# cgtuebingen/3D-RE-GEN

Hardware: AMD Instinct MI355X
Metric: objects/sec (50-step Hunyuan3D-2 DiT + 256^3 marching cubes) (higher is better)
Workload: dtype bf16; 1 GPU; configs[1]: 5 synthetic 512x512 RGBA crops per GPU, Hunyuan3D-2 full dims bf16, 50 flow-matching steps x CFG 2, 257^3 grid query + Lewiner marching cubes; weights=seeded synthetic, objects_total=5, objects_per_launch=4, parallelism=object-parallel x1

## Files before the change

3d-re-gen_amd/csrc/attn.hip:

```cpp
#include <hip/hip_runtime.h>
#include <cstdio>
#include <cstring>
#include <stddef.h>
#include <stdint.h>

#include <type_traits>

#include "kernels.h"
#include "prof.h"

namespace r3g {
namespace {

typedef __attribute__((ext_vector_type(8))) __bf16 bf16x8;
typedef __attribute__((ext_vector_type(4))) __bf16 bf16x4;
typedef __attribute__((ext_vector_type(16))) float f32x16;
typedef __attribute__((ext_vector_type(8))) float f32x8;

constexpr int KV_TILE = 64;
constexpr int TILE_B = KV_TILE * 64 * 2;
constexpr int STAGE_B = 2 * TILE_B;

typedef __attribute__((ext_vector_type(2))) __bf16 bf16x2;
typedef __attribute__((ext_vector_type(2))) float f32x2;
// ... 791 lines not shown
                m_run = half_max(mx);
#pragma unroll
                for (int r = 0; r < 16; ++r) { negm[r] = -m_run; s[r] -= m_run; }
            } else if (!kFast && __any(q < Lq && !(mx <= SCORE_LIMIT))) {
                const float grow = fmaxf(half_max(mx), 0.f);
                const float alpha = __builtin_amdgcn_exp2f(-grow);
                m_run += grow;
                l_run *= alpha;
#pragma unroll
                for (int r = 0; r < 16; ++r) { o[0][r] *= alpha; o[1][r] *= alpha; negm[r] -= grow; s[r] -= grow; }
            }
            float pe[16];
            uint32_t pk[8];
#pragma unroll
            for (int r = 0; r < 16; ++r) pe[r] = (ABL & 1) ? s[r] * 0.001f : __builtin_amdgcn_exp2f(s[r]);
#pragma unroll
            for (int e = 0; e < 8; ++e) pk[e] = pack_bf16(pe[2 * e], pe[2 * e + 1]);
            {
                const float psum = sum16(pe);
                l_run += psum;
                if (kFast && !first_block) sticky |= __ballot(!(psum <= PSUM_LIMIT2)) & valid_lanes;
            }
#pragma unroll
            for (int ks2 = 0; ks2 < 2; ++ks2) {
                union { uint32_t u[4]; bf16x8 v; } pf;
#pragma unroll
                for (int e = 0; e < 4; ++e) pf.u[e] = pk[4 * ks2 + e];
#pragma unroll
                for (int db = 0; db < 2; ++db) {
                    const bf16x8 vf = (ABL & 64) ? qf[(ks2 + db) & 3]
                                                 : *reinterpret_cast<const bf16x8*>(cur + TILE_B + (off[db] ^ ((2 * kb + ks2) << 5)));
                    if (ABL & 4) asm volatile("" ::"v"(vf), "v"(pf.v));
                    else o[db] = __builtin_amdgcn_mfma_f32_32x32x16_bf16(vf, pf.v, o[db], 0, 0, 0);
                }
            }
        }
        if (!(ABL & 32)) {
            asm volatile("s_waitcnt vmcnt(0)" ::: "memory");
            __syncthreads();
        }
    };
    if (ntiles == 1) {
        if (pad_tail) tile(std::true_type{}, std::true_type{}, 0);
        else tile(std::false_type{}, std::true_type{}, 0);
    } else {
        tile(std::false_type{}, std::true_type{}, 0);
        for (int t = 1; t < ntiles - 1; ++t) tile(std::false_type{}, std::false_type{}, t);
        if (pad_tail) tile(std::true_type{}, std::false_type{}, ntiles - 1);
        else tile(std::false_type{}, std::false_type{}, ntiles - 1);
    }
    };
    if constexpr ((VAR & 1) != 0 && ABL == 0) {
        pass(std::true_type{});
        if (__syncthreads_or(sticky != 0)) pass(std::false_type{});
    } else {
        pass(std::false_type{});
    }
    }

    const float inv = 1.0f / half_sum(l_run);
    {
        int64_t orow = (int64_t)b * p.strideO + (int64_t)q * p.ldo;
        if (p.ragged) orow = attn_entry_out_row(eb, q) * p.ldo;
        uint16_t* dst = p.O + orow + hd * 64;
#pragma unroll
        for (int db = 0; db < 2; ++db)
#pragma unroll
            for (int gp = 0; gp < 2; ++gp) {
                uint2 even, odd;
                even.x = pack_bf16(o[db][8 * gp] * inv, o[db][8 * gp + 1] * inv);
                even.y = pack_bf16(o[db][8 * gp + 2] * inv, o[db][8 * gp + 3] * inv);
                odd.x = pack_bf16(o[db][8 * gp + 4] * inv, o[db][8 * gp + 5] * inv);
                odd.y = pack_bf16(o[db][8 * gp + 6] * inv, o[db][8 * gp + 7] * inv);
                const u32x2 rx = __builtin_amdgcn_permlane32_swap(even.x, odd.x, false, false);
                const u32x2 ry = __builtin_amdgcn_permlane32_swap(even.y, odd.y, false, false);
                uint4 out;
                out.x = rx[0]; out.y = ry[0]; out.z = rx[1]; out.w = ry[1];
                if (q < Lq) *reinterpret_cast<uint4*>(dst + db * 32 + 16 * gp + 8 * hh) = out;
            }
    }
}

struct SoftmaxRun { float ps0, ps1, ea, eb; };
template <int J>
__device__ __forceinline__ void softmax_step(f32x8& half, uint32_t (&pk)[8], SoftmaxRun& st) {
    asm volatile("" : "+v"(half));
    const float a = __builtin_amdgcn_exp2f(half[2 * (J & 3)]);
    const float b = __builtin_amdgcn_exp2f(half[2 * (J & 3) + 1]);
    if (J == 1) { st.ps0 = st.ea; st.ps1 = st.eb; }
    if (J > 1) { st.ps0 += st.ea; st.ps1 += st.eb; }
    if (J > 0) {
        pk[J - 1] = pack_bf16(st.ea, st.eb);
        asm volatile("" : "+v"(pk[J - 1]));
    }
    st.ea = a;
    st.eb = b;
    if (J == 7) {
        pk[7] = pack_bf16(a, b);
        st.ps0 += a;
        st.ps1 += b;
        asm volatile("" : "+v"(pk[7]));
    }
    asm volatile("" : "+v"(st.ps0), "+v"(st.ps1), "+v"(st.ea), "+v"(st.eb));
}

template <int NW, int VAR = 0>
__global__ __launch_bounds__(NW * 64, 2) void attn3_kernel(AttnArgs p) {
    __shared__ __attribute__((aligned(16))) char smem[2 * STAGE_B];
    const int tid = threadIdx.x, lane = tid & 63;
    const int wid = __builtin_amdgcn_readfirstlane(tid >> 6);
    const int ql = lane & 31, hh = lane >> 5;
    constexpr int QT = NW * 64;
    int eb, hd, qt;
    {
        const int nwg = gridDim.x, orig = blockIdx.x;
        const int qn = nwg >> 3, rn = nwg & 7, xcd = orig & 7;
        const int item = (xcd < rn ? xcd * (qn + 1) : rn * (qn + 1) + (xcd - rn) * qn) + (orig >> 3);
        attn_work_item<QT>(p, item, eb, hd, qt);
    }
    const AttnEntry en = attn_entry(p, eb);
    const int b = en.buf;
    const int q0 = qt * QT + wid * 64 + ql;
    const int Lq = en.lq, Lk = en.lk;
    const int kvb = p.kv_batch_stride_zero ? 0 : b;
    const uint16_t* Qg = p.Q + (((int64_t)b * p.H + hd) * p.Lq_pad) * 64;
    const uint16_t* Kg = p.K + (((int64_t)kvb * p.H + hd) * p.Lk_pad) * 64;
    const uint16_t* Vtg = p.Vt + (((int64_t)kvb * p.H + hd) * 64) * (int64_t)p.Lk_pad;

    bf16x8 qf[2][4];
#pragma unroll
    for (int qb = 0; qb < 2; ++qb) {
        const int q = q0 + qb * 32;
        const int qrow = q < p.Lq_pad ? q : p.Lq_pad - 1;
#pragma unroll
        for (int ks = 0; ks < 4; ++ks)
            qf[qb][ks] = *reinterpret_cast<const bf16x8*>(Qg + (int64_t)qrow * 64 + ks * 16 + hh * 8);
    }
    if (!p.q_prescaled) {
        const float sc = p.scale * 1.4426950408889634f;
#pragma unroll
        for (int qb = 0; qb < 2; ++qb)
#pragma unroll
            for (int ks = 0; ks < 4; ++ks) {
                union { bf16x8 v; uint32_t u[4]; } w;
                w.v = qf[qb][ks];
#pragma unroll
                for (int e = 0; e < 4; ++e)
                    w.u[e] = pack_bf16(__uint_as_float(w.u[e] << 16) * sc, __uint_as_float(w.u[e] & 0xFFFF0000u) * sc);
                qf[qb][ks] = w.v;
            }
    }

    f32x16 o[2][2], negm[2];
    float m_run[2], l_run[2];
    unsigned long long sticky = 0;
    const unsigned long long valid_lanes[2] = {__ballot(q0 < Lq), __ballot(q0 + 32 < Lq)};

    int off[2];
#pragma unroll
    for (int rb = 0; rb < 2; ++rb) {
        const int row = rb * 32 + ql;
        off[rb] = row * 128 + ((hh ^ ((row >> 1) & 7)) << 4);
    }

    const int ntiles = (Lk + KV_TILE - 1) / KV_TILE;
    const int bias_key = en.bias_key;
    const float bias_l2 = p.ragged ? en.bias_log2 : 0.f;
    constexpr int PPW = 8 / NW;
    uint32_t koff[PPW], voff[PPW];
#pragma unroll
    for (int i = 0; i < PPW; ++i) {
        const int row = (wid * PPW + i) * 8 + (lane >> 3);
        const int kc = (lane & 7) ^ ((row >> 1) & 7);
        koff[i] = (uint32_t)(row * 64 + kc * 8) * 2u;
        voff[i] = ((uint32_t)row * (uint32_t)p.Lk_pad + (uint32_t)(kc * 8)) * 2u;
    }
    const uint32_t smem_lds = lds_address(smem);
    auto stage = [&](int t, char* dst) {
        const char* kt = reinterpret_cast<const char*>(Kg + (int64_t)t * (KV_TILE * 64));
        const char* vt = reinterpret_cast<const char*>(Vtg + (int64_t)t * KV_TILE);
#pragma unroll
        for (int i = 0; i < PPW; ++i) {
            if constexpr ((VAR & 4) != 0) {
                lds_dma16_unseen(kt, koff[i], smem_lds + (uint32_t)(dst - smem) + (wid * PPW + i) * 1024);
                lds_dma16_unseen(vt, voff[i], smem_lds + (uint32_t)(dst - smem) + TILE_B + (wid * PPW + i) * 1024);
                continue;
            }
            __builtin_amdgcn_global_load_lds((const __attribute__((address_space(1))) void*)(kt + (size_t)koff[i]),
                                             (__attribute__((address_space(3))) void*)(dst + (wid * PPW + i) * 1024), 16, 0, 0);
            __builtin_amdgcn_global_load_lds((const __attribute__((address_space(1))) void*)(vt + (size_t)voff[i]),
                                             (__attribute__((address_space(3))) void*)(dst + TILE_B + (wid * PPW + i) * 1024),
                                             16, 0, 0);
        }
    };
    const bool pad_tail = ntiles * KV_TILE > Lk;
    auto pass = [&](auto FAST) __attribute__((always_inline)) {
    constexpr bool kFast = decltype(FAST)::value;
#pragma unroll
    for (int qb = 0; qb < 2; ++qb) {
#pragma unroll
        for (int r = 0; r < 16; ++r) { o[qb][0][r] = 0.f; o[qb][1][r] = 0.f; negm[qb][r] = 0.f; }
        m_run[qb] = 0.f;
        l_run[qb] = 0.f;
    }
    stage(0, smem);
    asm volatile("s_waitcnt vmcnt(0)" ::: "memory");
    __syncthreads();

    auto tile = [&](auto masked, auto first, const int t) {
        const char* cur = smem + (t & 1) * STAGE_B;
        if constexpr ((VAR & 4) != 0) __builtin_amdgcn_s_waitcnt(0x0F70);
        if (t + 1 < ntiles) stage(t + 1, smem + ((t + 1) & 1) * STAGE_B);
        if constexpr ((VAR & 2) != 0 && kFast && !decltype(masked)::value && !decltype(first)::value) {
            auto ldk = [&](int kb, int ks) { return *reinterpret_cast<const bf16x8*>(cur + (off[kb] ^ (ks << 5))); };
            auto ldv = [&](int kb, int i) {
                return *reinterpret_cast<const bf16x8*>(cur + TILE_B + (off[i & 1] ^ ((2 * kb + (i >> 1)) << 5)));
            };
            auto pfrag = [&](const uint32_t (&pk)[8], int ks2) {
                union { uint32_t u[4]; bf16x8 v; } pf;
#pragma unroll
                for (int e = 0; e < 4; ++e) pf.u[e] = pk[4 * ks2 + e];
                return pf.v;
            };
            auto finish = [&](int qb, const SoftmaxRun& ps) {
                const float psum = ps.ps0 + ps.ps1;
                l_run[qb] += psum;
                sticky |= __ballot(!(psum <= PSUM_LIMIT2)) & valid_lanes[qb];
            };
#define R3G_GAP() __builtin_amdgcn_sched_barrier(0)
            f32x16 s00, s10, s01, s11;
            uint32_t pk00[8], pk10[8], pk01[8], pk11[8];
            SoftmaxRun ps;
            f32x8 h;
            bf16x8 fa[4], fb[4], fc[4], fd[4], fe[4], ff[4];
#pragma unroll
            for (int i = 0; i < 4; ++i) fa[i] = ldk(0, i);
            s00 = mfma_32x32x16_fresh(fa[0], qf[0][0], negm[0]); R3G_GAP();
            s00 = __builtin_amdgcn_mfma_f32_32x32x16_bf16(fa[1], qf[0][1], s00, 0, 0, 0); R3G_GAP();
            s00 = __builtin_amdgcn_mfma_f32_32x32x16_bf16(fa[2], qf[0][2], s00, 0, 0, 0); R3G_GAP();
            s00 = __builtin_amdgcn_mfma_f32_32x32x16_bf16(fa[3], qf[0][3], s00, 0, 0, 0); R3G_GAP();
            s10 = mfma_32x32x16_fresh(fa[0], qf[1][0], negm[1]); h = s00.lo; softmax_step<0>(h, pk00, ps); R3G_GAP();
            s10 = __builtin_amdgcn_mfma_f32_32x32x16_bf16(fa[1], qf[1][1], s10, 0, 0, 0); softmax_step<1>(h, pk00, ps); R3G_GAP();
            s10 = __builtin_amdgcn_mfma_f32_32x32x16_bf16(fa[2], qf[1][2], s10, 0, 0, 0); softmax_step<2>(h, pk00, ps); fb[0] = ldk(1, 0); R3G_GAP();
            s10 = __builtin_amdgcn_mfma_f32_32x32x16_bf16(fa[3], qf[1][3], s10, 0, 0, 0); softmax_step<3>(h, pk00, ps); fb[1] = ldk(1, 1); R3G_GAP();
            s01 = mfma_32x32x16_fresh(fb[0], qf[0][0], negm[0]); h = s00.hi; softmax_step<4>(h, pk00, ps); fb[2] = ldk(1, 2); R3G_GAP();
            s01 = __builtin_amdgcn_mfma_f32_32x32x16_bf16(fb[1], qf[0][1], s01, 0, 0, 0); softmax_step<5>(h, pk00, ps); fb[3] = ldk(1, 3); R3G_GAP();
            s01 = __builtin_amdgcn_mfma_f32_32x32x16_bf16(fb[2], qf[0][2], s01, 0, 0, 0); softmax_step<6>(h, pk00, ps); fc[0] = ldv(0, 0); R3G_GAP();
            s01 = __builtin_amdgcn_mfma_f32_32x32x16_bf16(fb[3], qf[0][3], s01, 0, 0, 0); softmax_step<7>(h, pk00, ps); fc[1] = ldv(0, 1); finish(0, ps); R3G_GAP();
            o[0][0] = __builtin_amdgcn_mfma_f32_32x32x16_bf16(fc[0], pfrag(pk00, 0), o[0][0], 0, 0, 0); h = s10.lo; softmax_step<0>(h, pk10, ps); fc[2] = ldv(0, 2); R3G_GAP();
            o[0][1] = __builtin_amdgcn_mfma_f32_32x32x16_bf16(fc[1], pfrag(pk00, 0), o[0][1], 0, 0, 0); softmax_step<1>(h, pk10, ps); fc[3] = ldv(0, 3); R3G_GAP();
            o[0][0] = __builtin_amdgcn_mfma_f32_32x32x16_bf16(fc[2], pfrag(pk00, 1), o[0][0], 0, 0, 0); softmax_step<2>(h, pk10, ps); fd[0] = ldk(1, 0); R3G_GAP();
            o[0][1] = __builtin_amdgcn_mfma_f32_32x32x16_bf16(fc[3], pfrag(pk00, 1), o[0][1], 0, 0, 0); softmax_step<3>(h, pk10, ps); fd[1] = ldk(1, 1); R3G_GAP();
            s11 = mfma_32x32x16_fresh(fd[0], qf[1][0], negm[1]); h = s10.hi; softmax_step<4>(h, pk10, ps); fd[2] = ldk(1, 2); R3G_GAP();
            s11 = __builtin_amdgcn_mfma_f32_32x32x16_bf16(fd[1], qf[1][1], s11, 0, 0, 0); softmax_step<5>(h, pk10, ps); fd[3] = ldk(1, 3); R3G_GAP();
            s11 = __builtin_amdgcn_mfma_f32_32x32x16_bf16(fd[2], qf[1][2], s11, 0, 0, 0); softmax_step<6>(h, pk10, ps); fe[0] = ldv(0, 0); R3G_GAP();
            s11 = __builtin_amdgcn_mfma_f32_32x32x16_bf16(fd[3], qf[1][3], s11, 0, 0, 0); softmax_step<7>(h, pk10, ps); fe[1] = ldv(0, 1); finish(1, ps); R3G_GAP();
            o[1][0] = __builtin_amdgcn_mfma_f32_32x32x16_bf16(fe[0], pfrag(pk10, 0), o[1][0], 0, 0, 0); h = s01.lo; softmax_step<0>(h, pk01, ps); fe[2] = ldv(0, 2); R3G_GAP();
            o[1][1] = __builtin_amdgcn_mfma_f32_32x32x16_bf16(fe[1], pfrag(pk10, 0), o[1][1], 0, 0, 0); softmax_step<1>(h, pk01, ps); fe[3] = ldv(0, 3); R3G_GAP();
            o[1][0] = __builtin_amdgcn_mfma_f32_32x32x16_bf16(fe[2], pfrag(pk10, 1), o[1][0], 0, 0, 0); softmax_step<2>(h, pk01, ps); ff[0] = ldv(1, 0); R3G_GAP();
            o[1][1] = __builtin_amdgcn_mfma_f32_32x32x16_bf16(fe[3], pfrag(pk10, 1), o[1][1], 0, 0, 0); softmax_step<3>(h, pk01, ps); ff[1] = ldv(1, 1); R3G_GAP();
            ff[2] = ldv(1, 2); ff[3] = ldv(1, 3);
            h = s01.hi; softmax_step<4>(h, pk01, ps); softmax_step<5>(h, pk01, ps); softmax_step<6>(h, pk01, ps); softmax_step<7>(h, pk01, ps); finish(0, ps); R3G_GAP();
            o[0][0] = __builtin_amdgcn_mfma_f32_32x32x16_bf16(ff[0], pfrag(pk01, 0), o[0][0], 0, 0, 0); h = s11.lo; softmax_step<0>(h, pk11, ps); R3G_GAP();
            o[0][1] = __builtin_amdgcn_mfma_f32_32x32x16_bf16(ff[1], pfrag(pk01, 0), o[0][1], 0, 0, 0); softmax_step<1>(h, pk11, ps); R3G_GAP();
            o[0][0] = __builtin_amdgcn_mfma_f32_32x32x16_bf16(ff[2], pfrag(pk01, 1), o[0][0], 0, 0, 0); softmax_step<2>(h, pk11, ps); R3G_GAP();
            o[0][1] = __builtin_amdgcn_mfma_f32_32x32x16_bf16(ff[3], pfrag(pk01, 1), o[0][1], 0, 0, 0); softmax_step<3>(h, pk11, ps); R3G_GAP();
            h = s11.hi; softmax_step<4>(h, pk11, ps); softmax_step<5>(h, pk11, ps); softmax_step<6>(h, pk11, ps); softmax_step<7>(h, pk11, ps); finish(1, ps); R3G_GAP();
            o[1][0] = __builtin_amdgcn_mfma_f32_32x32x16_bf16(ff[0], pfrag(pk11, 0), o[1][0], 0, 0, 0);
            o[1][1] = __builtin_amdgcn_mfma_f32_32x32x16_bf16(ff[1], pfrag(pk11, 0), o[1][1], 0, 0, 0);
            o[1][0] = __builtin_amdgcn_mfma_f32_32x32x16_bf16(ff[2], pfrag(pk11, 1), o[1][0], 0, 0, 0);
            o[1][1] = __builtin_amdgcn_mfma_f32_32x32x16_bf16(ff[3], pfrag(pk11, 1), o[1][1], 0, 0, 0);
#undef R3G_GAP
        } else {
#pragma unroll
        for (int kb = 0; kb < 2; ++kb) {
            constexpr bool kFirst = decltype(first)::value;
            const bool first_block = kFirst && kb == 0;
            bf16x8 kf[4];
#pragma unroll
            for (int ks = 0; ks < 4; ++ks) kf[ks] = *reinterpret_cast<const bf16x8*>(cur + (off[kb] ^ (ks << 5)));
            f32x16 s[2];
            if (first_block) {
                f32x16 z;
#pragma unroll
                for (int r = 0; r < 16; ++r) z[r] = 0.f;
                s[0] = __builtin_amdgcn_mfma_f32_32x32x16_bf16(kf[0], qf[0][0], z, 0, 0, 0);
                s[1] = __builtin_amdgcn_mfma_f32_32x32x16_bf16(kf[0], qf[1][0], z, 0, 0, 0);
            } else {
                s[0] = mfma_32x32x16_fresh(kf[0], qf[0][0], negm[0]);
                s[1] = mfma_32x32x16_fresh(kf[0], qf[1][0], negm[1]);
            }
#pragma unroll
            for (int ks = 1; ks < 4; ++ks) {
                s[0] = __builtin_amdgcn_mfma_f32_32x32x16_bf16(kf[ks], qf[0][ks], s[0], 0, 0, 0);
                s[1] = __builtin_amdgcn_mfma_f32_32x32x16_bf16(kf[ks], qf[1][ks], s[1], 0, 0, 0);
            }
            uint32_t pk[2][8];
#pragma unroll
            for (int qb = 0; qb < 2; ++qb) {
                f32x16& sq = s[qb];
                if constexpr (decltype(masked)::value) {
                    const int key_base = t * KV_TILE + kb * 32 + 4 * hh;
#pragma unroll
                    for (int r = 0; r < 16; ++r) {
                        const int key = key_base + (r & 3) + 8 * (r >> 2);
                        if (key >= Lk) sq[r] = -INFINITY;
                        else if (key == bias_key) sq[r] += bias_l2;
                    }
                }
                float mx = 0.f;
                if (first_block || !kFast) {
                    mx = fmaxf(sq[0], sq[1]);
#pragma unroll
                    for (int r = 2; r < 16; r += 2) mx = fmaxf(fmaxf(mx, sq[r]), sq[r + 1]);
                }
                if (first_block) {
                    m_run[qb] = half_max(mx);
#pragma unroll
                    for (int r = 0; r < 16; ++r) { negm[qb][r] = -m_run[qb]; sq[r] -= m_run[qb]; }
                } else if (!kFast && __any(q0 + qb * 32 < Lq && !(mx <= SCORE_LIMIT))) {
                    const float grow = fmaxf(half_max(mx), 0.f);
                    const float alpha = __builtin_amdgcn_exp2f(-grow);
                    m_run[qb] += grow;
                    l_run[qb] *= alpha;
#pragma unroll
                    for (int r = 0; r < 16; ++r) {
                        o[qb][0][r] *= alpha;
                        o[qb][1][r] *= alpha;
                        negm[qb][r] -= grow;
                        sq[r] -= grow;
                    }
                }
                float pe[16];
#pragma unroll
                for (int r = 0; r < 16; ++r) pe[r] = __builtin_amdgcn_exp2f(sq[r]);
#pragma unroll
                for (int e = 0; e < 8; ++e) pk[qb][e] = pack_bf16(pe[2 * e], pe[2 * e + 1]);
                const float psum = sum16(pe);
                l_run[qb] += psum;
                if (kFast && !first_block) sticky |= __ballot(!(psum <= PSUM_LIMIT2)) & valid_lanes[qb];
            }
#pragma unroll
            for (int ks2 = 0; ks2 < 2; ++ks2) {
                union { uint32_t u[4]; bf16x8 v; } pf[2];
#pragma unroll
                for (int qb = 0; qb < 2; ++qb)
#pragma unroll
                    for (int e = 0; e < 4; ++e) pf[qb].u[e] = pk[qb][4 * ks2 + e];
#pragma unroll
                for (int db = 0; db < 2; ++db) {
                    const bf16x8 vf = *reinterpret_cast<const bf16x8*>(cur + TILE_B + (off[db] ^ ((2 * kb + ks2) << 5)));
                    o[0][db] = __builtin_amdgcn_mfma_f32_32x32x16_bf16(vf, pf[0].v, o[0][db], 0, 0, 0);
                    o[1][db] = __builtin_amdgcn_mfma_f32_32x32x16_bf16(vf, pf[1].v, o[1][db], 0, 0, 0);
                }
            }
        }
        }
        asm volatile("s_waitcnt vmcnt(0)" ::: "memory");
        __syncthreads();
    };
    if (ntiles == 1) {
        if (pad_tail) tile(std::true_type{}, std::true_type{}, 0);
        else tile(std::false_type{}, std::true_type{}, 0);
    } else {
        tile(std::false_type{}, std::true_type{}, 0);
        for (int t = 1; t < ntiles - 1; ++t) tile(std::false_type{}, std::false_type{}, t);
        if (pad_tail) tile(std::true_type{}, std::false_type{}, ntiles - 1);
        else tile(std::false_type{}, std::false_type{}, ntiles - 1);
    }
    };
    if constexpr ((VAR & 1) != 0) {
        pass(std::true_type{});
        if (__syncthreads_or(sticky != 0)) pass(std::false_type{});
    } else {
        pass(std::false_type{});
    }

#pragma unroll
    for (int qb = 0; qb < 2; ++qb) {
        const int q = q0 + qb * 32;
        const float inv = 1.0f / half_sum(l_run[qb]);
        int64_t orow = (int64_t)b * p.strideO + (int64_t)q * p.ldo;
        if (p.ragged) orow = attn_entry_out_row(eb, q) * p.ldo;
        uint16_t* dst = p.O + orow + hd * 64;
#pragma unroll
        for (int db = 0; db < 2; ++db)
#pragma unroll
            for (int gp = 0; gp < 2; ++gp) {
                uint2 even, odd;
                even.x = pack_bf16(o[qb][db][8 * gp] * inv, o[qb][db][8 * gp + 1] * inv);
                even.y = pack_bf16(o[qb][db][8 * gp + 2] * inv, o[qb][db][8 * gp + 3] * inv);
                odd.x = pack_bf16(o[qb][db][8 * gp + 4] * inv, o[qb][db][8 * gp + 5] * inv);
                odd.y = pack_bf16(o[qb][db][8 * gp + 6] * inv, o[qb][db][8 * gp + 7] * inv);
                const u32x2 rx = __builtin_amdgcn_permlane32_swap(even.x, odd.x, false, false);
                const u32x2 ry = __builtin_amdgcn_permlane32_swap(even.y, odd.y, false, false);
                uint4 out;
                out.x = rx[0]; out.y = ry[0]; out.z = rx[1]; out.w = ry[1];
                if (q < Lq) *reinterpret_cast<uint4*>(dst + db * 32 + 16 * gp + 8 * hh) = out;
            }
    }
}


template <bool STAMP, int PRIO>
__global__ __launch_bounds__(768, 3) void attn6_kernel(AttnArgs p, unsigned long long* __restrict__ stamps) {
    extern __shared__ __attribute__((aligned(16))) char smem6[];
    char* const smem = smem6;
    constexpr int R = 4;
    const int tid = threadIdx.x, lane = tid & 63;
    const int wid = __builtin_amdgcn_readfirstlane(tid >> 6);
    const int grp = wid >> 2;
    const int ql = lane & 31, hh = lane >> 5;
    constexpr int QT = 384;
    int eb, hd, qt;
    {
        const int nwg = gridDim.x, orig = blockIdx.x;
        const int qn = nwg >> 3, rn = nwg & 7, xcd = orig & 7;
        const int item = (xcd < rn ? xcd * (qn + 1) : rn * (qn + 1) + (xcd - rn) * qn) + (orig >> 3);
        attn_work_item<QT>(p, item, eb, hd, qt);
    }
    const AttnEntry en = attn_entry(p, eb);
    const int b = en.buf;
    const int q = qt * QT + wid * 32 + ql;
    const int Lq = en.lq, Lk = en.lk;
    const int kvb = p.kv_batch_stride_zero ? 0 : b;
    const uint16_t* Qg = p.Q + (((int64_t)b * p.H + hd) * p.Lq_pad) * 64;
    const uint16_t* Kg = p.K + (((int64_t)kvb * p.H + hd) * p.Lk_pad) * 64;
    const uint16_t* Vtg = p.Vt + (((int64_t)kvb * p.H + hd) * 64) * (int64_t)p.Lk_pad;

    const int ntiles = (Lk + KV_TILE - 1) / KV_TILE;
    const int nblk = 2 * ntiles;
    const bool stager = wid < 8;
    int koff, voff;
    {
        const int row = (wid & 7) * 8 + (lane >> 3);
        const int kc = (lane & 7) ^ ((row >> 1) & 7);
        koff = row * 64 + kc * 8;
        voff = row * p.Lk_pad + kc * 8;
    }
    auto stage = [&](int t) {
        char* dst = smem + (t % R) * STAGE_B;
        const uint16_t* kt = Kg + (int64_t)t * (KV_TILE * 64);
        const uint16_t* vt = Vtg + (int64_t)t * KV_TILE;
        __builtin_amdgcn_global_load_lds((const __attribute__((address_space(1))) void*)(kt + koff),
                                         (__attribute__((address_space(3))) void*)(dst + (wid & 7) * 1024), 16, 0, 0);
        __builtin_amdgcn_global_load_lds((const __attribute__((address_space(1))) void*)(vt + voff),
                                         (__attribute__((address_space(3))) void*)(dst + TILE_B + (wid & 7) * 1024), 16, 0, 0);
    };
    auto wait_tile = [&](int u) {
        if (u + 1 < ntiles) asm volatile("s_waitcnt vmcnt(2)" ::: "memory");
        else asm volatile("s_waitcnt vmcnt(0)" ::: "memory");
    };
    if (stager) {
        stage(0);
        if (ntiles > 1) stage(1);
    }
    bf16x8 qf[4];
    {
        const int qrow = q < p.Lq_pad ? q : p.Lq_pad - 1;
#pragma unroll
        for (int ks = 0; ks < 4; ++ks)
            qf[ks] = *reinterpret_cast<const bf16x8*>(Qg + (int64_t)qrow * 64 + ks * 16 + hh * 8);
    }
    if (!p.q_prescaled) {
        const float sc = p.scale * 1.4426950408889634f;
#pragma unroll
        for (int ks = 0; ks < 4; ++ks) {
            union { bf16x8 v; uint32_t u[4]; } w;
            w.v = qf[ks];
#pragma unroll
            for (int e = 0; e < 4; ++e)
                w.u[e] = pack_bf16(__uint_as_float(w.u[e] << 16) * sc, __uint_as_float(w.u[e] & 0xFFFF0000u) * sc);
            qf[ks] = w.v;
        }
    }
    f32x16 o[2], negm;
#pragma unroll
    for (int r = 0; r < 16; ++r) { o[0][r] = 0.f; o[1][r] = 0.f; negm[r] = 0.f; }
    float m_run = 0.f, l_run = 0.f;
    int off[2];
#pragma unroll
    for (int rb = 0; rb < 2; ++rb) {
        const int row = rb * 32 + ql;
        off[rb] = row * 128 + ((hh ^ ((row >> 1) & 7)) << 4);
// ... 81 lines not shown
        {
            f32x2 ps = (f32x2){pe[0], pe[1]};
#pragma unroll
            for (int r = 2; r < 16; r += 2) ps += (f32x2){pe[r], pe[r + 1]};
            l_run += ps[0] + ps[1];
        }
        asm volatile("" : "+v"(pk[0]), "+v"(pk[1]), "+v"(pk[2]), "+v"(pk[3]), "+v"(pk[4]), "+v"(pk[5]), "+v"(pk[6]), "+v"(pk[7]),
                          "+v"(l_run));
        asm volatile("s_waitcnt lgkmcnt(0)" ::: "memory");
        if (PRIO == 2) __builtin_amdgcn_s_setprio(0);
        R3G_PHASE_END();
        if (PRIO == 1) __builtin_amdgcn_s_setprio(1);
        {
            union { uint32_t u[4]; bf16x8 v; } pf0, pf1;
#pragma unroll
            for (int e = 0; e < 4; ++e) { pf0.u[e] = pk[e]; pf1.u[e] = pk[4 + e]; }
            s_next = mfma_32x32x16_fresh(kf[0], qf[0], negm);
            o[0] = __builtin_amdgcn_mfma_f32_32x32x16_bf16(vf[0][0], pf0.v, o[0], 0, 0, 0);
            s_next = __builtin_amdgcn_mfma_f32_32x32x16_bf16(kf[1], qf[1], s_next, 0, 0, 0);
            o[1] = __builtin_amdgcn_mfma_f32_32x32x16_bf16(vf[0][1], pf0.v, o[1], 0, 0, 0);
            s_next = __builtin_amdgcn_mfma_f32_32x32x16_bf16(kf[2], qf[2], s_next, 0, 0, 0);
            o[0] = __builtin_amdgcn_mfma_f32_32x32x16_bf16(vf[1][0], pf1.v, o[0], 0, 0, 0);
            s_next = __builtin_amdgcn_mfma_f32_32x32x16_bf16(kf[3], qf[3], s_next, 0, 0, 0);
            o[1] = __builtin_amdgcn_mfma_f32_32x32x16_bf16(vf[1][1], pf1.v, o[1], 0, 0, 0);
        }
        if (PRIO == 1) __builtin_amdgcn_s_setprio(0);
        if (kb == 0 && grp == 1) wait_tile(t + 1);
        R3G_PHASE_END();
    };
    if (STAMP) {
#pragma unroll
        for (int k = 0; k < 6; ++k) st_acc[k] = 0;
        st_ph = 0;
        st_t0 = __builtin_amdgcn_s_memtime();
    }
    for (int t = 0; t < ntiles; ++t) {
        block(std::integral_constant<int, 0>{}, t, sA, sB);
        block(std::integral_constant<int, 1>{}, t, sB, sA);
    }
    if (STAMP && lane == 0 && stamps) {
#pragma unroll
        for (int k = 0; k < 6; ++k) atomicAdd(&stamps[grp * 8 + k], st_acc[k]);
        atomicAdd(&stamps[grp * 8 + 6], (unsigned long long)nblk);
    }

    const float inv = 1.0f / half_sum(l_run);
    {
        int64_t orow = (int64_t)b * p.strideO + (int64_t)q * p.ldo;
        if (p.ragged) orow = attn_entry_out_row(eb, q) * p.ldo;
        uint16_t* dst = p.O + orow + hd * 64;
#pragma unroll
        for (int db = 0; db < 2; ++db)
#pragma unroll
            for (int gp = 0; gp < 2; ++gp) {
                uint2 even, odd;
                even.x = pack_bf16(o[db][8 * gp] * inv, o[db][8 * gp + 1] * inv);
                even.y = pack_bf16(o[db][8 * gp + 2] * inv, o[db][8 * gp + 3] * inv);
                odd.x = pack_bf16(o[db][8 * gp + 4] * inv, o[db][8 * gp + 5] * inv);
                odd.y = pack_bf16(o[db][8 * gp + 6] * inv, o[db][8 * gp + 7] * inv);
                const u32x2 rx = __builtin_amdgcn_permlane32_swap(even.x, odd.x, false, false);
                const u32x2 ry = __builtin_amdgcn_permlane32_swap(even.y, odd.y, false, false);
                uint4 out;
                out.x = rx[0]; out.y = ry[0]; out.z = rx[1]; out.w = ry[1];
                if (q < Lq) *reinterpret_cast<uint4*>(dst + db * 32 + 16 * gp + 8 * hh) = out;
            }
    }
    for (int g = grp; g < 2; ++g) R3G_PHASE_END();
#undef R3G_PHASE_END
}

}

static bool g_attn_glds = true;
static bool g_attn_pipelined = false;
static int g_attn_ablate = 0;
void attn_set_ablate(int mask) { g_attn_ablate = mask; }
void attn_set_glds(bool on) { g_attn_glds = on; }
void attn_set_pipelined(bool on) { g_attn_pipelined = on; }

static int g_attn_gen = 7;
static int g_attn_variant = 1;
void attn_set_variant(int v) { if (v >= 0 && v <= 1) g_attn_variant = v; }
static int g_attn_interleave = 0;
void attn_set_interleave(int v) { g_attn_interleave = v != 0; }
static int g_attn_async_stage = 1;
void attn_set_async_stage(int v) { g_attn_async_stage = v != 0; }
static int g_wide6_min_items = 2048;
void attn_set_wide_min(int items) { if (items > 0) g_wide6_min_items = items; }
void attn_set_generation(int gen) { if ((gen >= 1 && gen <= 7) || gen == 9) g_attn_gen = gen; }
static int g_attn6_prio = 1;
void attn_set_prio(int v) { if (v >= 0 && v <= 2) g_attn6_prio = v; }
static int g_attn_stamps = 0;
void attn_set_stamps(int on) { g_attn_stamps = on; }

bool attn_glds() { return g_attn_glds; }
bool attn_get_option(const char* name, int* value) {
    if (!strcmp(name, "attn_variant")) *value = g_attn_variant;
    else if (!strcmp(name, "attn_interleave")) *value = g_attn_interleave;
    else if (!strcmp(name, "attn_async_stage")) *value = g_attn_async_stage;
    else if (!strcmp(name, "attn_pipelined")) *value = g_attn_pipelined ? 1 : 0;
    else if (!strcmp(name, "attn_ablate")) *value = g_attn_ablate;
    else if (!strcmp(name, "attn_generation")) *value = g_attn_gen;
    else if (!strcmp(name, "attn_stamps")) *value = g_attn_stamps;
    else if (!strcmp(name, "attn_prio")) *value = g_attn6_prio;
    else if (!strcmp(name, "attn_wide_min")) *value = g_wide6_min_items;
    else return false;
    return true;
}

float attn_q_scale(float scale) { return (g_attn_gen >= 2 && !g_attn_pipelined) ? scale * 1.4426950408889634f : 1.0f; }

hipError_t attention_launch(const AttnArgs& p, hipStream_t s) {
    if (p.ragged) {
        if (p.B < 1 || p.B > kAttnMaxEntries) return hipErrorInvalidValue;
        for (int b = 0; b < p.B; ++b) {
            const AttnEntry& en = p.ent[b];
            if (en.lq <= 0 || en.lk <= 0 || en.lq > p.Lq_pad || en.lk > p.Lk_pad || en.buf < 0) return hipErrorInvalidValue;
            const int nt = (en.lk + 63) / 64;
            if (en.bias_key >= 0 && (en.bias_key < (nt - 1) * 64 || nt * 64 == en.lk || en.bias_key >= en.lk))
                return hipErrorInvalidValue;
        }
    }
    if (p.Lq_pad % 128 || p.Lk_pad % 64 || p.Lk <= 0 || p.Lq <= 0 || p.Lk > p.Lk_pad || p.Lq > p.Lq_pad)
        return hipErrorInvalidValue;
    double pairs = (double)p.B * p.Lq * p.Lk;
    if (p.ragged) {
        pairs = 0;
        for (int b = 0; b < p.B; ++b) pairs += (double)p.ent[b].lq * p.ent[b].lk;
    }
    ProfScope ps(PC_ATTN, 4.0 * p.H * pairs * 64, s);
    if (g_attn_gen >= 2 && !g_attn_pipelined) {
        auto count = [&](int qtile) {
            int n = 0;
            if (p.ragged) for (int b = 0; b < p.B; ++b) n += (p.ent[b].lq + qtile - 1) / qtile;
            else n = ((p.Lq + qtile - 1) / qtile) * p.B;
            return n * p.H;
        };
        int gen = g_attn_gen;
        if (gen == 7) gen = (g_attn_glds && count(256) >= g_wide6_min_items) ? 6 : 2;
        const int qtile = (g_attn_glds && gen == 9) ? 384 : (g_attn_glds && gen >= 4) ? 256 : 128;
        const int items = count(qtile);
        if (!g_attn_glds) launch_count(LC_ATTN_REGISTER_STAGED);
        if (gen == 9 && g_attn_glds) {
            const int prio = g_attn6_prio;
            auto launch6 = [&](auto ST, unsigned long long* d_st) -> hipError_t {
                constexpr bool kSt = decltype(ST)::value;
                auto k0 = attn6_kernel<kSt, 0>;
                auto k1 = attn6_kernel<kSt, 1>;
                auto k2 = attn6_kernel<kSt, 2>;
                auto k = prio == 0 ? k0 : (prio == 2 ? k2 : k1);
                if (hipFuncSetAttribute((const void*)k, hipFuncAttributeMaxDynamicSharedMemorySize, 4 * STAGE_B) != hipSuccess) {
                    (void)hipGetLastError();
                    return hipErrorNotSupported;
                }
                launch_count(LC_ATTN_GEN9);
                hipLaunchKernelGGL(k, dim3(items), dim3(768), 4 * STAGE_B, s, p, d_st);
                return hipGetLastError();
            };
            if (g_attn_stamps) {
                static unsigned long long* d_st = nullptr;
                if (!d_st && hipMalloc((void**)&d_st, 24 * 8) != hipSuccess) return hipErrorOutOfMemory;
                (void)hipMemsetAsync(d_st, 0, 24 * 8, s);
                const hipError_t e = launch6(std::true_type{}, d_st);
                if (e != hipSuccess) return e;
                unsigned long long h[24];
                if (hipMemcpyAsync(h, d_st, sizeof(h), hipMemcpyDeviceToHost, s) != hipSuccess || hipStreamSynchronize(s) != hipSuccess)
                    return hipGetLastError();
                for (int g = 0; g < 3; ++g) {
                    const double n = (double)(h[g * 8 + 6] ? h[g * 8 + 6] : 1);
                    fprintf(stderr, "[attn6 stamps] prio %d group %d: ticks per block and wave: S1 %.0f + wait %.0f | S2 %.0f + wait %.0f | M %.0f + wait %.0f\n", prio, g,
                            h[g * 8] / n, h[g * 8 + 1] / n, h[g * 8 + 2] / n, h[g * 8 + 3] / n, h[g * 8 + 4] / n, h[g * 8 + 5] / n);
                }
                return hipSuccess;
            }
            return launch6(std::false_type{}, nullptr);
        }
        if (g_attn_ablate && gen == 2) {
            launch_count(LC_ATTN_GEN2);
            switch (g_attn_ablate) {
#define R3G_ABL2(m) case m: hipLaunchKernelGGL((attn2_kernel<true, false, 4, m>), dim3(items), dim3(256), 0, s, p); break;
                R3G_ABL2(1) R3G_ABL2(4) R3G_ABL2(8) R3G_ABL2(12) R3G_ABL2(16) R3G_ABL2(48) R3G_ABL2(64) R3G_ABL2(128)
                R3G_ABL2(192) R3G_ABL2(240) R3G_ABL2(241) R3G_ABL2(245) R3G_ABL2(253)
#undef R3G_ABL2
                default: return hipErrorInvalidValue;
            }
            return hipGetLastError();
        }
        launch_count(!g_attn_glds ? LC_ATTN_GEN2 : gen == 3 ? LC_ATTN_GEN3 : gen == 4 ? LC_ATTN_GEN4 : gen == 5 ? LC_ATTN_GEN5 : gen == 6 ? LC_ATTN_GEN6 : LC_ATTN_GEN2);
        if (!g_attn_glds) hipLaunchKernelGGL((attn2_kernel<false, false, 4>), dim3(items), dim3(256), 0, s, p);
        else if (gen == 3) hipLaunchKernelGGL((attn2_kernel<true, true, 4>), dim3(items), dim3(256), 0, s, p);
        else if (gen == 4) hipLaunchKernelGGL((attn2_kernel<true, true, 8>), dim3(items), dim3(512), 0, s, p);
        else if (gen == 5) hipLaunchKernelGGL((attn2_kernel<true, false, 8>), dim3(items), dim3(512), 0, s, p);
        else if (gen == 6) {
            if (g_attn_variant == 1) {
                switch ((g_attn_interleave ? 2 : 0) | (g_attn_async_stage ? 4 : 0)) {
                    case 6: hipLaunchKernelGGL((attn3_kernel<4, 7>), dim3(items), dim3(256), 0, s, p); break;
                    case 4: hipLaunchKernelGGL((attn3_kernel<4, 5>), dim3(items), dim3(256), 0, s, p); break;
                    case 2: hipLaunchKernelGGL((attn3_kernel<4, 3>), dim3(items), dim3(256), 0, s, p); break;
                    default: hipLaunchKernelGGL((attn3_kernel<4, 1>), dim3(items), dim3(256), 0, s, p); break;
                }
            }
            else hipLaunchKernelGGL((attn3_kernel<4, 0>), dim3(items), dim3(256), 0, s, p);
        } else {
            if (g_attn_variant == 1 && g_attn_async_stage) hipLaunchKernelGGL((attn2_kernel<true, false, 4, 0, 5>), dim3(items), dim3(256), 0, s, p);
            else if (g_attn_variant == 1) hipLaunchKernelGGL((attn2_kernel<true, false, 4, 0, 1>), dim3(items), dim3(256), 0, s, p);
            else hipLaunchKernelGGL((attn2_kernel<true, false, 4>), dim3(items), dim3(256), 0, s, p);
        }
        return hipGetLastError();
    }
    if (p.q_prescaled) return hipErrorInvalidValue;
    dim3 grid(p.Lq_pad / 128, p.H, p.B);
    launch_count(g_attn_pipelined ? LC_ATTN_PIPELINED : LC_ATTN_GEN1);
    if (!g_attn_glds) launch_count(LC_ATTN_REGISTER_STAGED);
    if (g_attn_pipelined) {
        if (g_attn_glds) hipLaunchKernelGGL(attn_kernel_sp<true>, grid, dim3(256), 0, s, p);
        else hipLaunchKernelGGL(attn_kernel_sp<false>, grid, dim3(256), 0, s, p);
    } else if (g_attn_glds && g_attn_ablate) {
        switch (g_attn_ablate) {
#define R3G_ABL(m) case m: hipLaunchKernelGGL((attn_kernel<true, m>), grid, dim3(256), 0, s, p); break;
            R3G_ABL(1) R3G_ABL(2) R3G_ABL(3) R3G_ABL(4) R3G_ABL(8) R3G_ABL(12) R3G_ABL(16) R3G_ABL(48) R3G_ABL(64) R3G_ABL(68)
            R3G_ABL(15) R3G_ABL(63) R3G_ABL(127)
#undef R3G_ABL
            default: return hipErrorInvalidValue;
        }
    } else if (g_attn_glds) {
        hipLaunchKernelGGL(attn_kernel<true>, grid, dim3(256), 0, s, p);
    } else {
        hipLaunchKernelGGL(attn_kernel<false>, grid, dim3(256), 0, s, p);
    }
    return hipGetLastError();
}

}
```

Baseline: 0.8052 objects/sec.

## Add skewed K/V software-pipelined attention body and route ragged mid-size shapes to it

Adds a skewed attn3 main loop that stages K and V separately. Each iteration overlaps the QK^T MFMAs of the next key block with the softmax and PV MFMAs of the previous one, with K one tile ahead of V. The launcher picks this body by default when the work-item count is large enough, including ragged mid-size cases that previously fell back to gen 2. For those moved cases it also adds a per-half safe-pass skip. This hides exp and pack latency behind matrix work, at the cost of more registers and complex tail handling that could hurt occupancy or correctness.

```diff
diff --git a/3d-re-gen_amd/csrc/attn.hip b/3d-re-gen_amd/csrc/attn.hip
--- a/3d-re-gen_amd/csrc/attn.hip
+++ b/3d-re-gen_amd/csrc/attn.hip
@@ -897,7 +897,7 @@
 }
 
 struct SoftmaxRun { float ps0, ps1, ea, eb; };
-template <int J>
+template <int J, bool TAIL = true>
 __device__ __forceinline__ void softmax_step(f32x8& half, uint32_t (&pk)[8], SoftmaxRun& st) {
     asm volatile("" : "+v"(half));
     const float a = __builtin_amdgcn_exp2f(half[2 * (J & 3)]);
@@ -910,13 +910,19 @@
     }
     st.ea = a;
     st.eb = b;
-    if (J == 7) {
+    if (J == 7 && TAIL) {
         pk[7] = pack_bf16(a, b);
         st.ps0 += a;
         st.ps1 += b;
         asm volatile("" : "+v"(pk[7]));
     }
     asm volatile("" : "+v"(st.ps0), "+v"(st.ps1), "+v"(st.ea), "+v"(st.eb));
+}
+__device__ __forceinline__ void softmax_tail(uint32_t (&pk)[8], SoftmaxRun& st) {
+    pk[7] = pack_bf16(st.ea, st.eb);
+    st.ps0 += st.ea;
+    st.ps1 += st.eb;
+    asm volatile("" : "+v"(pk[7]), "+v"(st.ps0), "+v"(st.ps1));
 }
 
 template <int NW, int VAR = 0>
@@ -991,26 +997,51 @@
         voff[i] = ((uint32_t)row * (uint32_t)p.Lk_pad + (uint32_t)(kc * 8)) * 2u;
     }
     const uint32_t smem_lds = lds_address(smem);
+    auto piece = [&](const char* base, uint32_t lane_off, char* dst) {
+        if constexpr ((VAR & 4) != 0)
+            lds_dma16_unseen(base, lane_off, smem_lds + (uint32_t)(dst - smem));
+        else
+            __builtin_amdgcn_global_load_lds((const __attribute__((address_space(1))) void*)(base + (size_t)lane_off),
+                                             (__attribute__((address_space(3))) void*)dst, 16, 0, 0);
+    };
     auto stage = [&](int t, char* dst) {
         const char* kt = reinterpret_cast<const char*>(Kg + (int64_t)t * (KV_TILE * 64));
         const char* vt = reinterpret_cast<const char*>(Vtg + (int64_t)t * KV_TILE);
 #pragma unroll
         for (int i = 0; i < PPW; ++i) {
-            if constexpr ((VAR & 4) != 0) {
-                lds_dma16_unseen(kt, koff[i], smem_lds + (uint32_t)(dst - smem) + (wid * PPW + i) * 1024);
-                lds_dma16_unseen(vt, voff[i], smem_lds + (uint32_t)(dst - smem) + TILE_B + (wid * PPW + i) * 1024);
-                continue;
-            }
-            __builtin_amdgcn_global_load_lds((const __attribute__((address_space(1))) void*)(kt + (size_t)koff[i]),
-                                             (__attribute__((address_space(3))) void*)(dst + (wid * PPW + i) * 1024), 16, 0, 0);
-            __builtin_amdgcn_global_load_lds((const __attribute__((address_space(1))) void*)(vt + (size_t)voff[i]),
-                                             (__attribute__((address_space(3))) void*)(dst + TILE_B + (wid * PPW + i) * 1024),
-                                             16, 0, 0);
-        }
+            piece(kt, koff[i], dst + (wid * PPW + i) * 1024);
+            piece(vt, voff[i], dst + TILE_B + (wid * PPW + i) * 1024);
+        }
+    };
+    auto stage_k = [&](int t, char* dst) {
+        const char* kt = reinterpret_cast<const char*>(Kg + (int64_t)t * (KV_TILE * 64));
+#pragma unroll
+        for (int i = 0; i < PPW; ++i) piece(kt, koff[i], dst + (wid * PPW + i) * 1024);
+    };
+    auto stage_v = [&](int t, char* dst) {
+        const char* vt = reinterpret_cast<const char*>(Vtg + (int64_t)t * KV_TILE);
+#pragma unroll
+        for (int i = 0; i < PPW; ++i) piece(vt, voff[i], dst + TILE_B + (wid * PPW + i) * 1024);
     };
     const bool pad_tail = ntiles * KV_TILE > Lk;
+    auto pfrag = [&](const uint32_t (&pk)[8], int ks2) {
+        union { uint32_t u[4]; bf16x8 v; } pf;
+#pragma unroll
+        for (int e = 0; e < 4; ++e) pf.u[e] = pk[4 * ks2 + e];
+        return pf.v;
+    };
+    auto finish = [&](int qb, const SoftmaxRun& ps) {
+        const float psum = ps.ps0 + ps.ps1;
+        l_run[qb] += psum;
+        sticky |= __ballot(!(psum <= PSUM_LIMIT2)) & valid_lanes[qb];
+    };
+#define R3G_GAP() __builtin_amdgcn_sched_barrier(0)
+    bool safe_active = true;
     auto pass = [&](auto FAST) __attribute__((always_inline)) {
     constexpr bool kFast = decltype(FAST)::value;
+    bool computes = true;
+    if constexpr (!kFast && (VAR & 16) != 0) computes = safe_active;
+    if (computes) {
 #pragma unroll
     for (int qb = 0; qb < 2; ++qb) {
 #pragma unroll
@@ -1018,31 +1049,19 @@
         m_run[qb] = 0.f;
         l_run[qb] = 0.f;
     }
-    stage(0, smem);
-    asm volatile("s_waitcnt vmcnt(0)" ::: "memory");
-    __syncthreads();
-
-    auto tile = [&](auto masked, auto first, const int t) {
+    }
+    auto tile = [&](auto masked, auto first, const int t, auto part) {
+        constexpr int kPart = decltype(part)::value;
         const char* cur = smem + (t & 1) * STAGE_B;
+        if constexpr (kPart == 0) {
         if constexpr ((VAR & 4) != 0) __builtin_amdgcn_s_waitcnt(0x0F70);
         if (t + 1 < ntiles) stage(t + 1, smem + ((t + 1) & 1) * STAGE_B);
+        }
         if constexpr ((VAR & 2) != 0 && kFast && !decltype(masked)::value && !decltype(first)::value) {
             auto ldk = [&](int kb, int ks) { return *reinterpret_cast<const bf16x8*>(cur + (off[kb] ^ (ks << 5))); };
             auto ldv = [&](int kb, int i) {
                 return *reinterpret_cast<const bf16x8*>(cur + TILE_B + (off[i & 1] ^ ((2 * kb + (i >> 1)) << 5)));
             };
-            auto pfrag = [&](const uint32_t (&pk)[8], int ks2) {
-                union { uint32_t u[4]; bf16x8 v; } pf;
-#pragma unroll
-                for (int e = 0; e < 4; ++e) pf.u[e] = pk[4 * ks2 + e];
-                return pf.v;
-            };
-            auto finish = [&](int qb, const SoftmaxRun& ps) {
-                const float psum = ps.ps0 + ps.ps1;
-                l_run[qb] += psum;
-                sticky |= __ballot(!(psum <= PSUM_LIMIT2)) & valid_lanes[qb];
-            };
-#define R3G_GAP() __builtin_amdgcn_sched_barrier(0)
             f32x16 s00, s10, s01, s11;
             uint32_t pk00[8], pk10[8], pk01[8], pk11[8];
             SoftmaxRun ps;
@@ -1085,10 +1104,9 @@
             o[1][1] = __builtin_amdgcn_mfma_f32_32x32x16_bf16(ff[1], pfrag(pk11, 0), o[1][1], 0, 0, 0);
             o[1][0] = __builtin_amdgcn_mfma_f32_32x32x16_bf16(ff[2], pfrag(pk11, 1), o[1][0], 0, 0, 0);
             o[1][1] = __builtin_amdgcn_mfma_f32_32x32x16_bf16(ff[3], pfrag(pk11, 1), o[1][1], 0, 0, 0);
-#undef R3G_GAP
-        } else {
-#pragma unroll
-        for (int kb = 0; kb < 2; ++kb) {
+        } else if (computes) {
+#pragma unroll
+        for (int kb = 0; kb < (kPart == 1 ? 1 : 2); ++kb) {
             constexpr bool kFirst = decltype(first)::value;
             const bool first_block = kFirst && kb == 0;
             bf16x8 kf[4];
@@ -1171,22 +1189,151 @@
             }
         }
         }
+        if constexpr (kPart == 1) return;
         asm volatile("s_waitcnt vmcnt(0)" ::: "memory");
         __syncthreads();
     };
+    constexpr std::integral_constant<int, 0> whole{};
+
+    constexpr bool kSkewed = (VAR & 8) != 0 && kFast;
+    if constexpr (kSkewed) if (ntiles >= 2) {
+        auto ldk = [&](const char* st, int kb, int ks) { return *reinterpret_cast<const bf16x8*>(st + (off[kb] ^ (ks << 5))); };
+        auto ldv = [&](const char* st, int kb, int i) {
+            return *reinterpret_cast<const bf16x8*>(st + TILE_B + (off[i & 1] ^ ((2 * kb + (i >> 1)) << 5)));
+        };
+        auto landed = [&]() {
+            asm volatile("s_waitcnt vmcnt(0)" ::: "memory");
+            __syncthreads();
+            if constexpr ((VAR & 4) != 0) __builtin_amdgcn_s_waitcnt(0x0F70);
+        };
+        char* const st0 = smem;
+        char* const st1 = smem + STAGE_B;
+        stage_k(0, st0); stage_v(0, st0); stage_k(1, st1);
+        landed();
+        stage_v(1, st1);
+        tile(std::false_type{}, std::true_type{}, 0, std::integral_constant<int, 1>{});
+
+        f32x16 s0, s1;
+        uint32_t pk0[8], pk1[8];
+        bf16x8 kf[4], vf[4];
+        SoftmaxRun ps;
+        f32x8 h;
+#pragma unroll
+        for (int ks = 0; ks < 4; ++ks) kf[ks] = ldk(st0, 1, ks);
+        s0 = mfma_32x32x16_fresh(kf[0], qf[0][0], negm[0]);
+        s1 = mfma_32x32x16_fresh(kf[0], qf[1][0], negm[1]);
+#pragma unroll
+        for (int ks = 1; ks < 4; ++ks) {
+            s0 = __builtin_amdgcn_mfma_f32_32x32x16_bf16(kf[ks], qf[0][ks], s0, 0, 0, 0);
+            s1 = __builtin_amdgcn_mfma_f32_32x32x16_bf16(kf[ks], qf[1][ks], s1, 0, 0, 0);
+        }
+        __syncthreads();
+        if (2 < ntiles) stage_k(2, st0);
+#pragma unroll
+        for (int ks = 0; ks < 4; ++ks) kf[ks] = ldk(st1, 0, ks);
+        h = s0.lo; softmax_step<0>(h, pk0, ps); softmax_step<1>(h, pk0, ps); softmax_step<2>(h, pk0, ps); softmax_step<3>(h, pk0, ps);
+        h = s0.hi; softmax_step<4>(h, pk0, ps); softmax_step<5>(h, pk0, ps); softmax_step<6>(h, pk0, ps); softmax_step<7, false>(h, pk0, ps);
+
+        auto iteration = [&](auto VS, auto VKB, auto KS, auto KKB) {
+            const char* const vst = smem + decltype(VS)::value * STAGE_B;
+            const char* const kst = smem + decltype(KS)::value * STAGE_B;
+            constexpr int vkb = decltype(VKB)::value, kkb = decltype(KKB)::value;
+            R3G_GAP();
+            s0 = mfma_32x32x16_fresh(kf[0], qf[0][0], negm[0]); R3G_GAP();
+            softmax_tail(pk0, ps); h = s1.lo; softmax_step<0>(h, pk1, ps); vf[0] = ldv(vst, vkb, 0); R3G_GAP();
+            s0 = __builtin_amdgcn_mfma_f32_32x32x16_bf16(kf[1], qf[0][1], s0, 0, 0, 0); R3G_GAP();
+            finish(0, ps); softmax_step<1>(h, pk1, ps); vf[1] = ldv(vst, vkb, 1); R3G_GAP();
+            s0 = __builtin_amdgcn_mfma_f32_32x32x16_bf16(kf[2], qf[0][2], s0, 0, 0, 0); R3G_GAP();
+            softmax_step<2>(h, pk1, ps); vf[2] = ldv(vst, vkb, 2); R3G_GAP();
+            s0 = __builtin_amdgcn_mfma_f32_32x32x16_bf16(kf[3], qf[0][3], s0, 0, 0, 0); R3G_GAP();
+            softmax_step<3>(h, pk1, ps); vf[3] = ldv(vst, vkb, 3); R3G_GAP();
+            o[0][0] = __builtin_amdgcn_mfma_f32_32x32x16_bf16(vf[0], pfrag(pk0, 0), o[0][0], 0, 0, 0); R3G_GAP();
+            h = s1.hi; softmax_step<4>(h, pk1, ps); R3G_GAP();
+            o[0][1] = __builtin_amdgcn_mfma_f32_32x32x16_bf16(vf[1], pfrag(pk0, 0), o[0][1], 0, 0, 0); R3G_GAP();
+            softmax_step<5>(h, pk1, ps); R3G_GAP();
+            o[0][0] = __builtin_amdgcn_mfma_f32_32x32x16_bf16(vf[2], pfrag(pk0, 1), o[0][0], 0, 0, 0); R3G_GAP();
+            softmax_step<6>(h, pk1, ps); R3G_GAP();
+            o[0][1] = __builtin_amdgcn_mfma_f32_32x32x16_bf16(vf[3], pfrag(pk0, 1), o[0][1], 0, 0, 0); R3G_GAP();
+            softmax_step<7, false>(h, pk1, ps); R3G_GAP();
+            s1 = mfma_32x32x16_fresh(kf[0], qf[1][0], negm[1]); R3G_GAP();
+            softmax_tail(pk1, ps); h = s0.lo; softmax_step<0>(h, pk0, ps); R3G_GAP();
+            s1 = __builtin_amdgcn_mfma_f32_32x32x16_bf16(kf[1], qf[1][1], s1, 0, 0, 0); R3G_GAP();
+            finish(1, ps); softmax_step<1>(h, pk0, ps); R3G_GAP();
+            s1 = __builtin_amdgcn_mfma_f32_32x32x16_bf16(kf[2], qf[1][2], s1, 0, 0, 0); R3G_GAP();
+            softmax_step<2>(h, pk0, ps); R3G_GAP();
+            s1 = __builtin_amdgcn_mfma_f32_32x32x16_bf16(kf[3], qf[1][3], s1, 0, 0, 0); R3G_GAP();
+            softmax_step<3>(h, pk0, ps); R3G_GAP();
+            o[1][0] = __builtin_amdgcn_mfma_f32_32x32x16_bf16(vf[0], pfrag(pk1, 0), o[1][0], 0, 0, 0); R3G_GAP();
+            h = s0.hi; softmax_step<4>(h, pk0, ps); kf[0] = ldk(kst, kkb, 0); R3G_GAP();
+            o[1][1] = __builtin_amdgcn_mfma_f32_32x32x16_bf16(vf[1], pfrag(pk1, 0), o[1][1], 0, 0, 0); R3G_GAP();
+            softmax_step<5>(h, pk0, ps); kf[1] = ldk(kst, kkb, 1); R3G_GAP();
+            o[1][0] = __builtin_amdgcn_mfma_f32_32x32x16_bf16(vf[2], pfrag(pk1, 1), o[1][0], 0, 0, 0); R3G_GAP();
+            softmax_step<6>(h, pk0, ps); kf[2] = ldk(kst, kkb, 2); R3G_GAP();
+            o[1][1] = __builtin_amdgcn_mfma_f32_32x32x16_bf16(vf[3], pfrag(pk1, 1), o[1][1], 0, 0, 0); R3G_GAP();
+            softmax_step<7, false>(h, pk0, ps); kf[3] = ldk(kst, kkb, 3); R3G_GAP();
+        };
+        auto trip = [&](auto P, const int T) {
+            constexpr std::integral_constant<int, decltype(P)::value> a{};
+            constexpr std::integral_constant<int, 1 - decltype(P)::value> b{};
+            constexpr std::integral_constant<int, 0> kb0{};
+            constexpr std::integral_constant<int, 1> kb1{};
+            iteration(a, kb1, b, kb1);
+            landed();
+            if (T + 3 < ntiles) stage_k(T + 3, smem + b.value * STAGE_B);
+            if (T + 2 < ntiles) stage_v(T + 2, smem + a.value * STAGE_B);
+            iteration(b, kb0, a, kb0);
+        };
+        const int ntrips = pad_tail ? ntiles - 2 : ntiles - 1;
+        int T = 0;
+        for (; T + 2 <= ntrips; T += 2) {
+            trip(std::integral_constant<int, 0>{}, T);
+            trip(std::integral_constant<int, 1>{}, T + 1);
+        }
+        if (T < ntrips) trip(std::integral_constant<int, 0>{}, T);
+        {
+            const char* sl = smem + (ntrips & 1) * STAGE_B;
+#pragma unroll
+            for (int i = 0; i < 4; ++i) vf[i] = ldv(sl, 1, i);
+            softmax_tail(pk0, ps);
+            finish(0, ps);
+            h = s1.lo; softmax_step<0>(h, pk1, ps); softmax_step<1>(h, pk1, ps); softmax_step<2>(h, pk1, ps); softmax_step<3>(h, pk1, ps);
+            h = s1.hi; softmax_step<4>(h, pk1, ps); softmax_step<5>(h, pk1, ps); softmax_step<6>(h, pk1, ps); softmax_step<7>(h, pk1, ps);
+            finish(1, ps);
+#pragma unroll
+            for (int i = 0; i < 4; ++i) {
+                o[0][i & 1] = __builtin_amdgcn_mfma_f32_32x32x16_bf16(vf[i], pfrag(pk0, i >> 1), o[0][i & 1], 0, 0, 0);
+                o[1][i & 1] = __builtin_amdgcn_mfma_f32_32x32x16_bf16(vf[i], pfrag(pk1, i >> 1), o[1][i & 1], 0, 0, 0);
+            }
+        }
+        if (pad_tail) {
+            landed();
+            tile(std::true_type{}, std::false_type{}, ntiles - 1, std::integral_constant<int, 2>{});
+        }
+        return;
+    }
+
+    stage(0, smem);
+    asm volatile("s_waitcnt vmcnt(0)" ::: "memory");
+    __syncthreads();
     if (ntiles == 1) {
-        if (pad_tail) tile(std::true_type{}, std::true_type{}, 0);
-        else tile(std::false_type{}, std::true_type{}, 0);
-    } else {
-        tile(std::false_type{}, std::true_type{}, 0);
-        for (int t = 1; t < ntiles - 1; ++t) tile(std::false_type{}, std::false_type{}, t);
-        if (pad_tail) tile(std::true_type{}, std::false_type{}, ntiles - 1);
-        else tile(std::false_type{}, std::false_type{}, ntiles - 1);
+        if (pad_tail) tile(std::true_type{}, std::true_type{}, 0, whole);
+        else tile(std::false_type{}, std::true_type{}, 0, whole);
+    } else if constexpr (!kSkewed) {
+        tile(std::false_type{}, std::true_type{}, 0, whole);
+        for (int t = 1; t < ntiles - 1; ++t) tile(std::false_type{}, std::false_type{}, t, whole);
+        if (pad_tail) tile(std::true_type{}, std::false_type{}, ntiles - 1, whole);
+        else tile(std::false_type{}, std::false_type{}, ntiles - 1, whole);
     }
     };
     if constexpr ((VAR & 1) != 0) {
         pass(std::true_type{});
-        if (__syncthreads_or(sticky != 0)) pass(std::false_type{});
+        if constexpr ((VAR & 16) != 0) {
+            const int lo = __syncthreads_or(sticky != 0 && wid < NW / 2), hi = __syncthreads_or(sticky != 0 && wid >= NW / 2);
+            if (lo | hi) {
+                safe_active = __builtin_amdgcn_readfirstlane(wid < NW / 2 ? lo : hi) != 0;
+                pass(std::false_type{});
+            }
+        } else if (__syncthreads_or(sticky != 0)) pass(std::false_type{});
     } else {
         pass(std::false_type{});
     }
@@ -1215,6 +1362,7 @@
             }
     }
 }
+#undef R3G_GAP
 
 
 template <bool STAMP, int PRIO>
@@ -1462,7 +1610,7 @@
 static int g_attn_variant = 1;
 void attn_set_variant(int v) { if (v >= 0 && v <= 1) g_attn_variant = v; }
 static int g_attn_interleave = 0;
-void attn_set_interleave(int v) { g_attn_interleave = v != 0; }
+void attn_set_interleave(int v) { if (v >= 0 && v <= 3) g_attn_interleave = v; }
 static int g_attn_async_stage = 1;
 void attn_set_async_stage(int v) { g_attn_async_stage = v != 0; }
 static int g_wide6_min_items = 2048;
@@ -1490,6 +1638,17 @@
 
 float attn_q_scale(float scale) { return (g_attn_gen >= 2 && !g_attn_pipelined) ? scale * 1.4426950408889634f : 1.0f; }
 
+constexpr int kSkewMinItems = 2048, kSkewMinItemsRagged = 1024;
+static bool attn3_skew_pays(const AttnArgs& p, int items) { return items >= kSkewMinItems || (p.ragged && items >= kSkewMinItemsRagged); }
+static int attn3_body(const AttnArgs& p, int items) {
+    switch (g_attn_interleave) {
+        case 0: return attn3_skew_pays(p, items) ? 8 : 0;
+        case 1: return 2;
+        case 2: return 8;
+        default: return 0;
+    }
+}
+
 hipError_t attention_launch(const AttnArgs& p, hipStream_t s) {
     if (p.ragged) {
         if (p.B < 1 || p.B > kAttnMaxEntries) return hipErrorInvalidValue;
@@ -1517,7 +1676,13 @@
             return n * p.H;
         };
         int gen = g_attn_gen;
-        if (gen == 7) gen = (g_attn_glds && count(256) >= g_wide6_min_items) ? 6 : 2;
+        bool moved = false;
+        if (gen == 7) {
+            const int wide_items = count(256);
+            const bool wide = wide_items >= g_wide6_min_items;
+            moved = !wide && p.ragged && g_attn_interleave == 0 && g_attn_variant == 1 && wide_items >= kSkewMinItemsRagged;
+            gen = (g_attn_glds && (wide || moved)) ? 6 : 2;
+        }
         const int qtile = (g_attn_glds && gen == 9) ? 384 : (g_attn_glds && gen >= 4) ? 256 : 128;
         const int items = count(qtile);
         if (!g_attn_glds) launch_count(LC_ATTN_REGISTER_STAGED);
@@ -1573,7 +1738,11 @@
         else if (gen == 5) hipLaunchKernelGGL((attn2_kernel<true, false, 8>), dim3(items), dim3(512), 0, s, p);
         else if (gen == 6) {
             if (g_attn_variant == 1) {
-                switch ((g_attn_interleave ? 2 : 0) | (g_attn_async_stage ? 4 : 0)) {
+                switch (attn3_body(p, items) | (g_attn_async_stage ? 4 : 0) | (moved && g_attn_glds ? 16 : 0)) {
+                    case 28: hipLaunchKernelGGL((attn3_kernel<4, 29>), dim3(items), dim3(256), 0, s, p); break;
+                    case 24: hipLaunchKernelGGL((attn3_kernel<4, 25>), dim3(items), dim3(256), 0, s, p); break;
+                    case 12: hipLaunchKernelGGL((attn3_kernel<4, 13>), dim3(items), dim3(256), 0, s, p); break;
+                    case 8: hipLaunchKernelGGL((attn3_kernel<4, 9>), dim3(items), dim3(256), 0, s, p); break;
                     case 6: hipLaunchKernelGGL((attn3_kernel<4, 7>), dim3(items), dim3(256), 0, s, p); break;
                     case 4: hipLaunchKernelGGL((attn3_kernel<4, 5>), dim3(items), dim3(256), 0, s, p); break;
                     case 2: hipLaunchKernelGGL((attn3_kernel<4, 3>), dim3(items), dim3(256), 0, s, p); break;
```

Result: faster. 0.8284 objects/sec, median of 6 (+2.9%).
